# HySonLab/Protein_Redesign

Hardware: AMD Instinct MI355X
Metric: denoising-steps/sec (fwd+rev) per complex, N=256 res (higher is better)
Workload: dtype f32; 1 GPU; configs[1]: synthetic 256-residue + 64-atom ligand (N=320), single_dim=512 pair_dim=64 num_blocks=4 num_steps=1000, 1 complex/GPU, sharded by sample index (no data-path collective; one all_gather of the samples at the end of the timed region); samples_per_gpu=1, hip_graph=True, outputs_finite=True, backend=single process

## Files before the change

### protein_redesign_amd/csrc/prd_tri.hip

```cpp
#include "prd_common.h"
#include "../../include/prd_hip.h"
#include <atomic>
#include <cstdlib>
#include <cstring>
#include "prd_launch.h"

#ifdef PRD_TIMING
__device__ unsigned long long prd_dbg[256 * 16 * 8 * 4];
__device__ int prd_dbg_sel;
extern "C" int prd_debug_read(void* dst) { return (int)hipMemcpyFromSymbol(dst, HIP_SYMBOL(prd_dbg), sizeof(prd_dbg)); }
extern "C" int prd_debug_select(int id) { return (int)hipMemcpyToSymbol(HIP_SYMBOL(prd_dbg_sel), &id, sizeof(int)); }
#define PRD_STAMP(k) do { if (lane == 0 && it < 8) prd_dbg[((blockIdx.x * 12 + wave) * 8 + it) * 4 + (k)] = __builtin_readcyclecounter(); } while (0)
struct PhaseTimer {
    unsigned long long t, acc[8];
    __device__ PhaseTimer() { for (int k = 0; k < 8; ++k) acc[k] = 0; t = __builtin_readcyclecounter(); }
    __device__ void mark(int k) {
        __builtin_amdgcn_sched_barrier(0);
        const unsigned long long n = __builtin_readcyclecounter();
        __builtin_amdgcn_sched_barrier(0);
        acc[k] += n - t;
        t = n;
    }
    __device__ void flush(int id = 0) {
        if (prd_dbg_sel != 0 && prd_dbg_sel != id) return;
        if ((threadIdx.x & 63) == 0) for (int k = 0; k < 8; ++k) prd_dbg[(blockIdx.x * 16 + (threadIdx.x >> 6)) * 8 + k] = acc[k];
    }
};
#else
#define PRD_STAMP(k)
struct PhaseTimer {
    __device__ void mark(int) {}
    __device__ void flush(int = 0) {}
};
#endif

namespace {

struct ProjTask {
    int ob, vb, bb, u, bu;
    bool ok;
};
template <int OB>
PRD_DEV ProjTask proj_decode(long task, int nrb, int nvb, int N) {
    ProjTask t;
    const int ti = task < 0 ? 0 : (int)task;
    const int grp = ti / (8 * OB), within = ti % (8 * OB);
    t.ob = within >> 3;
    int rb = grp * 8 + (within & 7);
    t.ok = task >= 0 && rb < nrb;
    if (!t.ok) rb = 0;
    t.vb = rb % nvb;
    t.bu = rb / nvb;
    t.bb = t.bu / N;
    t.u = t.bu - t.bb * N;
    return t;
}
template <int P>
PRD_DEV void proj_fetch(const ProjTask& t, const float* __restrict__ pair, const float* __restrict__ mask, int N, int incoming,
                        int r, int hi, float (&x)[P / 2], float& mu, float& mv) {
    const int v = t.vb * 32 + r;
    const bool valid = v < N;
    const int vv = valid ? v : 0;
    mu = mask[t.bu];
    mv = mask[t.bb * N + vv];
    const prd_rsrc rs = make_rsrc(pair + (long)t.bb * N * N * P);
    const unsigned rowi = incoming ? (unsigned)vv * N + t.u : (unsigned)t.u * N + vv;
    load_row_cll_buf<P>(rs, valid ? (rowi * P + 4 * hi) * 4u : BUF_OOB, x);
}

template <int P, bool B3>
PRD_DEV void proj_compute(const ProjTask& t, float (&x)[P / 2], float mu, float mv, float* __restrict__ AB,
                          const float* Wpl, const float* Wgl, const float* bpl, const float* bgl,
                          int N, int ldn, long cstride, unsigned lane_off, int r, int hi, PhaseTimer& pt) {
    constexpr int KH = P / 2, OUT = 2 * P;
    const bool valid = t.vb * 32 + r < N;
    pt.mark(0);
    const float m2 = valid ? mu * mv : 0.f;
    const bool plain = __all(m2 == 1.0f);
    pt.mark(1);
    ln_cll<KH>(x);
    pt.mark(2);
    f32x16 ap[1], ag[1];
    bias_acc(ap, bpl + hi * P + 16 * t.ob);
    bias_acc(ag, bgl + hi * P + 16 * t.ob);
    if (B3) {
        u32x4 xs[2][P / 16];
        split2h_cll<KH>(x, xs);
        rowgemm_h2<P, 1>(reinterpret_cast<const u32x4*>(Wpl), OUT, t.ob * 32, xs, ap, r, hi);
        rowgemm_h2<P, 1>(reinterpret_cast<const u32x4*>(Wgl), OUT, t.ob * 32, xs, ag, r, hi);
#pragma unroll
        for (int q = 0; q < 16; ++q) { ap[0][q] *= H2_INV_WSCALE; ag[0][q] *= H2_INV_WSCALE; }
    } else {
        rowgemm<P, 1>(Wpl + t.ob * 32 * (P + 4), x, ap, r, hi);
        rowgemm<P, 1>(Wgl + t.ob * 32 * (P + 4), x, ag, r, hi);
    }
    pt.mark(3);
    const prd_rsrc cb = make_rsrc(AB + ((((long)t.bb * 2 * P) + 32 * t.ob) * N + t.u) * ldn + t.vb * 32);
    const unsigned cbytes = (unsigned)cstride * 4u;
    if (plain) {
#pragma unroll
        for (int q = 0; q < 16; q += 2) {
            const f32x2 den = f32x2{__builtin_amdgcn_exp2f(ag[0][q]), __builtin_amdgcn_exp2f(ag[0][q + 1])} + 1.0f;
            const f32x2 val = f32x2{ap[0][q], ap[0][q + 1]} * f32x2{__builtin_amdgcn_rcpf(den.x), __builtin_amdgcn_rcpf(den.y)};
            buf_store(val.x, cb, lane_off, ((q & 3) + 8 * (q >> 2)) * cbytes);
            buf_store(val.y, cb, lane_off, (((q + 1) & 3) + 8 * ((q + 1) >> 2)) * cbytes);
        }
    } else {
#pragma unroll
        for (int q = 0; q < 16; ++q)
            buf_store(m2 * (gate_from_scaled(ag[0][q]) * ap[0][q]), cb, lane_off, ((q & 3) + 8 * (q >> 2)) * cbytes);
    }
    pt.mark(4);
}

size_t tri_mul_proj_lds_bytes(int P, bool b3) { return (2 * (b3 ? (size_t)2 * P * P : (size_t)2 * P * (P + 4)) + 4 * P) * sizeof(float); }
template <int P, int NW, bool B3>
__global__ __launch_bounds__(NW * 64) void tri_mul_proj_kernel(int* queue, float* __restrict__ AB, const float* __restrict__ pair,
                                                          const float* __restrict__ mask,
                                                          const float* __restrict__ wp, const float* __restrict__ bp,
                                                          const float* __restrict__ wg, const float* __restrict__ bg,
                                                          int b, int N, int ldn, int incoming) {
    constexpr int KH = P / 2, OUT = 2 * P, OB = OUT / 32;
    extern __shared__ __attribute__((aligned(16))) float smem[];
    PhaseTimer pt;
    constexpr int WSZ = B3 ? OUT * P : OUT * (P + 4);
    float* Wpl = smem;
    float* Wgl = Wpl + WSZ;
    float* bpl = Wgl + WSZ;
    float* bgl = bpl + OUT;
    if (B3) {
        stage_weight_h2<P>(reinterpret_cast<u32x4*>(Wpl), wp, OUT, P, threadIdx.x, NW * 64, H2_WSCALE);
        stage_weight_h2<P>(reinterpret_cast<u32x4*>(Wgl), wg, OUT, P, threadIdx.x, NW * 64, NEG_LOG2E * H2_WSCALE);
    } else {
        stage_weight_cll<P>(Wpl, wp, OUT, P, threadIdx.x, NW * 64);
        stage_weight_cll<P>(Wgl, wg, OUT, P, threadIdx.x, NW * 64, NEG_LOG2E);
    }
    stage_vec_cll(bpl, bp, OUT, threadIdx.x, NW * 64, B3 ? H2_WSCALE : 1.0f);
    stage_vec_cll(bgl, bg, OUT, threadIdx.x, NW * 64, NEG_LOG2E * (B3 ? H2_WSCALE : 1.0f));
    const int lane = threadIdx.x & 63, r = lane & 31, hi = lane >> 5;
    const int nvb = ldn / 32;
    const int nrb = b * N * nvb;
    const long ntask = (long)((nrb + 7) / 8 * 8) * OB;
    const long cstride = (long)N * ldn;
    const unsigned lane_off = (hi * 4 * (unsigned)cstride + r) * 4u;
    WaveTasks tasks(queue, ntask, NW);
    float xa[KH], xb[KH], mua, mva, mub, mvb;
    long t = tasks.next();
    ProjTask ta = proj_decode<OB>(t, nrb, nvb, N), tb;
    proj_fetch<P>(ta, pair, mask, N, incoming, r, hi, xa, mua, mva);
    __syncthreads();
    pt.mark(6);
    while (t >= 0) {
        const long tn = tasks.next();
        tb = proj_decode<OB>(tn, nrb, nvb, N);
        proj_fetch<P>(tb, pair, mask, N, incoming, r, hi, xb, mub, mvb);
        if (ta.ok) proj_compute<P, B3>(ta, xa, mua, mva, AB, Wpl, Wgl, bpl, bgl, N, ldn, cstride, lane_off, r, hi, pt);
        if (tn < 0) break;
        t = tasks.next();
        ta = proj_decode<OB>(t, nrb, nvb, N);
        proj_fetch<P>(ta, pair, mask, N, incoming, r, hi, xa, mua, mva);
        if (tb.ok) proj_compute<P, B3>(tb, xb, mub, mvb, AB, Wpl, Wgl, bpl, bgl, N, ldn, cstride, lane_off, r, hi, pt);
    }
    pt.mark(5);
    pt.flush(1);
}

size_t tri_mul_out_proj_lds_bytes(int P) { return ((size_t)2 * P * P + (size_t)2 * 2 * P * P + 6 * P) * sizeof(float); }
template <int P, int NW>
__global__ __launch_bounds__(NW * 64) void tri_mul_out_proj_kernel(float* pair, const float* __restrict__ Ot, const float* __restrict__ mask,
                                                                   const float* __restrict__ wo, const float* __restrict__ bo,
                                                                   const float* __restrict__ wog, const float* __restrict__ bog,
                                                                   const float* __restrict__ wp, const float* __restrict__ bp,
                                                                   const float* __restrict__ wg, const float* __restrict__ bg,
                                                                   float* __restrict__ AB, int b, int N, int ldn) {
    constexpr int KH = P / 2, NB = P / 32, OUT = 2 * P, OB = OUT / 32;
    extern __shared__ __attribute__((aligned(16))) float smem_op[];
    float* Wol = smem_op;
    float* Wgol = Wol + P * P;
    float* Wpl = Wgol + P * P;
    float* Wgl = Wpl + OUT * P;
    float* bol = Wgl + OUT * P;
    float* bgol = bol + P;
    float* bpl = bgol + P;
    float* bgl = bpl + OUT;
    stage_weight_h2<P>(reinterpret_cast<u32x4*>(Wol), wo, P, P, threadIdx.x, NW * 64, H2_WSCALE);
    stage_weight_h2<P>(reinterpret_cast<u32x4*>(Wgol), wog, P, P, threadIdx.x, NW * 64, H2_WSCALE);
    stage_weight_h2<P>(reinterpret_cast<u32x4*>(Wpl), wp, OUT, P, threadIdx.x, NW * 64, H2_WSCALE);
    stage_weight_h2<P>(reinterpret_cast<u32x4*>(Wgl), wg, OUT, P, threadIdx.x, NW * 64, NEG_LOG2E * H2_WSCALE);
    stage_vec_cll(bol, bo, P, threadIdx.x, NW * 64);
    stage_vec_cll(bgol, bog, P, threadIdx.x, NW * 64);
    stage_vec_cll(bpl, bp, OUT, threadIdx.x, NW * 64, H2_WSCALE);
    stage_vec_cll(bgl, bg, OUT, threadIdx.x, NW * 64, NEG_LOG2E * H2_WSCALE);
    __syncthreads();
    const int lane = threadIdx.x & 63, r_w = lane & 31, hi_w = lane >> 5;
    const int nvb = ldn / 32;
    const long ntask = (long)b * N * nvb;
    const unsigned cbytes = (unsigned)N * (unsigned)ldn * 4u;
    WaveTasks tasks(nullptr, ntask, NW);
    for (long task = tasks.next(); task >= 0; task = tasks.next()) {
        int r = r_w, hi = hi_w;
        asm volatile("" : "+v"(r), "+v"(hi));
        const unsigned lane_off = (unsigned)(4 * hi) * cbytes + (unsigned)r * 4u;
        const int ti = (int)task;
        const int vb = ti % nvb, bu = ti / nvb;
        const int bb = bu / N, u = bu - bb * N;
        const int v = vb * 32 + r;
        const bool valid = v < N;
        const int vv = valid ? v : 0;
        float x[KH], xr[KH];
        {
            const prd_rsrc ro = make_rsrc(Ot + (((long)bb * P) * N + u) * ldn + vb * 32);
#pragma unroll
            for (int s = 0; s < KH; ++s) x[s] = buf_load(ro, valid ? lane_off : BUF_OOB, (unsigned)(8 * (s >> 2) + (s & 3)) * cbytes);
            const prd_rsrc rp = make_rsrc(pair + (long)bb * N * N * P);
            load_row_cll_buf<P>(rp, valid ? (((unsigned)vv * N + u) * P + 4 * hi) * 4u : BUF_OOB, xr);
        }
        const float mu = mask[bu], mv = mask[bb * N + vv];
        float gate[KH];
        {
            float xn[KH];
#pragma unroll
            for (int s = 0; s < KH; ++s) xn[s] = xr[s];
            ln_cll<KH>(xn);
            f32x16 ag[NB];
            zero_acc(ag);
            u32x4 xs[2][P / 16];
            split2h_cll<KH>(xn, xs);
            rowgemm_h2<P, NB>(reinterpret_cast<const u32x4*>(Wgol), P, 0, xs, ag, r, hi);
#pragma unroll
            for (int s = 0; s < KH; ++s) gate[s] = sigmoid_fast(ag[s >> 4][s & 15] * H2_INV_WSCALE + bgol[hi * KH + s]);
        }
        ln_cll<KH>(x);
        {
            f32x16 ao[NB];
            zero_acc(ao);
            u32x4 xs[2][P / 16];
            split2h_cll<KH>(x, xs);
            rowgemm_h2<P, NB>(reinterpret_cast<const u32x4*>(Wol), P, 0, xs, ao, r, hi);
#pragma unroll
            for (int s = 0; s < KH; ++s) x[s] = xr[s] + gate[s] * (ao[s >> 4][s & 15] * H2_INV_WSCALE + bol[hi * KH + s]);
        }
        store_row_cll<P>(pair + (((long)bb * N + vv) * N + u) * P, hi, valid, x);
        ln_cll<KH>(x);
        u32x4 xs[2][P / 16];
        split2h_cll<KH>(x, xs);
        const float m2 = valid ? mu * mv : 0.f;
        const bool plain = __all(m2 == 1.0f);
#pragma unroll
        for (int ob = 0; ob < OB; ++ob) {
            f32x16 ap[1], ag[1];
            bias_acc(ap, bpl + hi * P + 16 * ob);
            bias_acc(ag, bgl + hi * P + 16 * ob);
            rowgemm_h2<P, 1>(reinterpret_cast<const u32x4*>(Wpl), OUT, ob * 32, xs, ap, r, hi);
            rowgemm_h2<P, 1>(reinterpret_cast<const u32x4*>(Wgl), OUT, ob * 32, xs, ag, r, hi);
            const prd_rsrc cb = make_rsrc(AB + ((((long)bb * 2 * P) + 32 * ob) * N + u) * ldn + vb * 32);
            if (plain) {
#pragma unroll
                for (int q = 0; q < 16; ++q) {
                    const float val = (ap[0][q] * H2_INV_WSCALE) * gate_from_scaled(ag[0][q] * H2_INV_WSCALE);
                    buf_store(val, cb, lane_off, (unsigned)((q & 3) + 8 * (q >> 2)) * cbytes);
                }
            } else {
#pragma unroll
                for (int q = 0; q < 16; ++q)
                    buf_store(m2 * ((ap[0][q] * H2_INV_WSCALE) * gate_from_scaled(ag[0][q] * H2_INV_WSCALE)), cb, lane_off,
                              (unsigned)((q & 3) + 8 * (q >> 2)) * cbytes);
            }
        }
    }
}

__global__ __launch_bounds__(256) void tri_mul_contract_kernel(float* __restrict__ O, const float* __restrict__ AB,
                                                               int N, int ldn, int P, int nbatch, int tiles) {
    constexpr int KCH = 32, LDP = KCH + 4;
    __shared__ __attribute__((aligned(16))) float As[2][64 * LDP];
    __shared__ __attribute__((aligned(16))) float Bs[2][64 * LDP];
    const int tid = threadIdx.x, lane = tid & 63, wave = tid >> 6;
    const int r = lane & 31, hi = lane >> 5;
    const int wm0 = (wave >> 1) * 32, wn0 = (wave & 1) * 32;
    const int nch = nbatch * P;
    const int t2 = tiles * tiles;
    for (int vblk = blockIdx.x; vblk < nch * t2; vblk += gridDim.x) {
    int ch, tile;
    if ((nch & 7) == 0 && (gridDim.x & 7) == 0) {
        const int xcd = vblk & 7, k = vblk >> 3;
        ch = xcd + 8 * (k / t2);
        tile = k % t2;
    } else {
        ch = vblk / t2;
        tile = vblk % t2;
    }
    const int bb = ch / P, d = ch - bb * P;
    const int m0 = (tile / tiles) * 64, n0 = (tile % tiles) * 64;
    const float* __restrict__ A = AB + ((size_t)bb * 2 * P + d) * N * ldn;
    const float* __restrict__ B = AB + ((size_t)bb * 2 * P + P + d) * N * ldn;
    const int srow = tid >> 3, sf = tid & 7;
    const bool a0 = (m0 + srow) < N, a1 = (m0 + srow + 32) < N, b0 = (n0 + srow) < N, b1 = (n0 + srow + 32) < N;
    const prd_rsrc ra = make_rsrc(A + (size_t)m0 * ldn), rb = make_rsrc(B + (size_t)n0 * ldn);
    const unsigned oa0 = a0 ? ((unsigned)srow * ldn + 4 * sf) * 4u : BUF_OOB, oa1 = a1 ? ((unsigned)(srow + 32) * ldn + 4 * sf) * 4u : BUF_OOB;
    const unsigned ob0 = b0 ? ((unsigned)srow * ldn + 4 * sf) * 4u : BUF_OOB, ob1 = b1 ? ((unsigned)(srow + 32) * ldn + 4 * sf) * 4u : BUF_OOB;
    f32x16 acc;
#pragma unroll
    for (int q = 0; q < 16; ++q) acc[q] = 0.f;
    const int nchunk = ldn / KCH;
#define PRD_TMC_LD1(RS, OFF, KO) [&] { const auto v_ = __builtin_amdgcn_raw_buffer_load_b128(RS, OFF, (KO) * 4, 0);      \
        return make_float4(__uint_as_float(v_[0]), __uint_as_float(v_[1]), __uint_as_float(v_[2]), __uint_as_float(v_[3])); }()
#define PRD_TMC_LOAD(R, KO)                                                       \
    R##a0 = PRD_TMC_LD1(ra, oa0, KO);                                             \
    R##a1 = PRD_TMC_LD1(ra, oa1, KO);                                             \
    R##b0 = PRD_TMC_LD1(rb, ob0, KO);                                             \
    R##b1 = PRD_TMC_LD1(rb, ob1, KO);
#define PRD_TMC_STAGE(R, BUF)                                                     \
    *reinterpret_cast<float4*>(&As[BUF][srow * LDP + 4 * sf]) = R##a0;            \
    *reinterpret_cast<float4*>(&As[BUF][(srow + 32) * LDP + 4 * sf]) = R##a1;     \
    *reinterpret_cast<float4*>(&Bs[BUF][srow * LDP + 4 * sf]) = R##b0;            \
    *reinterpret_cast<float4*>(&Bs[BUF][(srow + 32) * LDP + 4 * sf]) = R##b1;
#define PRD_TMC_CHUNK(C, CUR, R, N)                                               \
    {                                                                             \
        const int c2 = (C) + 2 < nchunk ? (C) + 2 : nchunk - 1;                   \
        PRD_TMC_LOAD(N, c2 * KCH)                                                 \
        const float* as = &As[CUR][(wm0 + r) * LDP + hi * 16];                    \
        const float* bs = &Bs[CUR][(wn0 + r) * LDP + hi * 16];                    \
        _Pragma("unroll") for (int t = 0; t < 4; ++t) {                           \
            const float4 a = *reinterpret_cast<const float4*>(as + 4 * t);        \
            const float4 bq = *reinterpret_cast<const float4*>(bs + 4 * t);       \
            acc = mfma32(a.x, bq.x, acc);                                         \
            acc = mfma32(a.y, bq.y, acc);                                         \
            acc = mfma32(a.z, bq.z, acc);                                         \
            acc = mfma32(a.w, bq.w, acc);                                         \
        }                                                                         \
        if ((C) + 1 < nchunk) { PRD_TMC_STAGE(R, (CUR) ^ 1) }                     \
        __syncthreads();                                                          \
    }
    float4 ua0, ua1, ub0, ub1, va0, va1, vb0, vb1;
    PRD_TMC_LOAD(u, 0)
    PRD_TMC_STAGE(u, 0)
    {
        const int c1 = 1 < nchunk ? 1 : 0;
        PRD_TMC_LOAD(u, c1 * KCH)
    }
    __syncthreads();
    for (int c = 0; c < nchunk; c += 2) {
        PRD_TMC_CHUNK(c, 0, u, v)
        if (c + 1 < nchunk) PRD_TMC_CHUNK(c + 1, 1, v, u)
    }
#undef PRD_TMC_LOAD
#undef PRD_TMC_LD1
#undef PRD_TMC_STAGE
#undef PRD_TMC_CHUNK
    float* __restrict__ Oc = O + (size_t)ch * N * ldn;
    const int n = n0 + wn0 + r;
    if (n < N) {
#pragma unroll
        for (int q = 0; q < 16; ++q) {
            const int m = m0 + wm0 + drow32(q, hi);
            if (m < N) Oc[(size_t)m * ldn + n] = acc[q];
        }
    }
    }
}

constexpr int TMS_T = 160, TMS_PLANE = TMS_T * 64, TMS_OPER = 2 * TMS_PLANE;
size_t tri_mul_contract_split_lds_bytes() { return (size_t)4 * TMS_OPER; }
template <int NWV, int DEPTH = 2, bool ASC = false>
__global__ __launch_bounds__(NWV * 64) void tri_mul_contract_split_kernel(float* __restrict__ O, const float* __restrict__ AB,
                                                                          int N, int ldn, int P, int nbatch, int tiles, int swap,
                                                                          const unsigned* __restrict__ a_amax) {
    constexpr int NT = NWV * 64, NPT = (2560 + NT - 1) / NT, NSUB = (25 + NWV - 1) / NWV;
    extern __shared__ __attribute__((aligned(16))) unsigned char tms[];
    PhaseTimer pt;
    const int tid = threadIdx.x, lane = tid & 63, wave = tid >> 6;
    const int r = lane & 31, hi = lane >> 5;
    const int nch = nbatch * P;
    const int t2 = tiles * tiles;
    unsigned srow[NPT], sdst[NPT], ssrc[NPT];
    bool sisb[NPT], sok[NPT];
    const int wbase = __builtin_amdgcn_readfirstlane(tid & ~63);
#pragma unroll
    for (int i = 0; i < NPT; ++i) {
        const int pw = wbase + NT * i;
        sok[i] = pw < 2560;
        const int oper = (sok[i] && pw >= 1280) ? 1 : 0;
        const int pc = sok[i] ? tid + NT * i : 0;
        const int q = pc - 1280 * oper;
        const int row = q >> 3, f = q & 7;
        sisb[i] = oper == 1;
        srow[i] = row;
        sdst[i] = oper * TMS_OPER + row * 64 + (((f >> 1) ^ ((row >> 2) & 3)) << 4) + (f & 1) * 8;
        ssrc[i] = ((unsigned)row * ldn + 4 * f) * 4u;
    }
    const unsigned swz = (unsigned)((r >> 2) & 3);
    for (int vblk = blockIdx.x; vblk < nch * t2; vblk += gridDim.x) {
        int ch, tile;
        if ((nch & 7) == 0 && (gridDim.x & 7) == 0) {
            const int xcd = vblk & 7, k = vblk >> 3;
            ch = xcd + 8 * (k / t2);
            tile = k % t2;
        } else {
            ch = vblk / t2;
            tile = vblk % t2;
        }
        const int bb = ch / P, d = ch - bb * P;
        const int m0 = (tile / tiles) * TMS_T, n0 = (tile % tiles) * TMS_T;
        float asc = 1.0f, iasc = 1.0f;
        if constexpr (ASC) {
            asc = split_scale(a_amax[bb]);
            iasc = __uint_as_float((254u << 23) - __float_as_uint(asc));
        }
        const float* __restrict__ A = AB + ((size_t)bb * 2 * P + (swap ? P : 0) + d) * N * ldn;
        const float* __restrict__ B = AB + ((size_t)bb * 2 * P + (swap ? 0 : P) + d) * N * ldn;
        const prd_rsrc ra = make_rsrc(A + (size_t)m0 * ldn), rb = make_rsrc(B + (size_t)n0 * ldn);
        unsigned off[NPT];
#pragma unroll
        for (int i = 0; i < NPT; ++i)
            off[i] = (sok[i] && (sisb[i] ? n0 : m0) + (int)srow[i] < N) ? ssrc[i] : BUF_OOB;
        int si[NSUB], sj[NSUB];
        bool sv[NSUB];
#pragma unroll
        for (int k = 0; k < NSUB; ++k) {
            const int s_ = wave + NWV * k;
            si[k] = s_ / 5;
            sj[k] = s_ - 5 * si[k];
            sv[k] = s_ < 25 && m0 + 32 * si[k] < N && n0 + 32 * sj[k] < N;
        }
        f32x16 acc[NSUB];
        zero_acc(acc);
        const int nchunk = ldn / 32;
        u32x4 u[NPT], v[NPT];
#define PRD_TMS_LOAD(R, C)                                                                                          \
    _Pragma("unroll") for (int i = 0; i < NPT; ++i)                                                                 \
        R[i] = __builtin_bit_cast(u32x4, __builtin_amdgcn_raw_buffer_load_b128(sisb[i] ? rb : ra, off[i], (C) * 128, 0));
#define PRD_TMS_STAGE(R, BUF)                                                                                       \
    _Pragma("unroll") for (int i = 0; i < NPT; ++i) {                                                               \
        if (!sok[i]) continue;                                                                                      \
        float x0 = __uint_as_float(R[i][0]), x1 = __uint_as_float(R[i][1]), x2 = __uint_as_float(R[i][2]), x3 = __uint_as_float(R[i][3]); \
        if (ASC && !sisb[i]) { x0 *= asc; x1 *= asc; x2 *= asc; x3 *= asc; }                                       \
        unsigned h0, l0, h1, l1;                                                                                    \
        split2h(x0, x1, h0, l0);                                                                                    \
        split2h(x2, x3, h1, l1);                                                                                    \
        unsigned char* dst = tms + (BUF) * 2 * TMS_OPER + sdst[i];                                                  \
        *reinterpret_cast<u32x2*>(dst) = u32x2{h0, h1};                                                             \
        *reinterpret_cast<u32x2*>(dst + TMS_PLANE) = u32x2{l0, l1};                                                 \
    }
#define PRD_TMS_CHUNK(C, CUR, R, NX)                                                                                \
    {                                                                                                               \
        const int c2 = (C) + 2 < nchunk ? (C) + 2 : nchunk - 1;                                                     \
        PRD_TMS_LOAD(NX, c2)                                                                                        \
        const unsigned char* base = tms + (CUR) * 2 * TMS_OPER;                                                     \
        _Pragma("unroll") for (int st = 0; st < 2; ++st) {                                                          \
            const unsigned col = (((unsigned)(2 * st + hi)) ^ swz) << 4;                                            \
            _Pragma("unroll") for (int k = 0; k < NSUB; ++k) {                                                      \
                if (sv[k]) {                                                                                        \
                    const unsigned char* ap = base + (32 * si[k] + r) * 64 + col;                                   \
                    const unsigned char* bp = base + TMS_OPER + (32 * sj[k] + r) * 64 + col;                        \
                    u32x4 a[2], bq[2];                                                                              \
                    _Pragma("unroll") for (int pl = 0; pl < 2; ++pl) {                                              \
                        a[pl] = *reinterpret_cast<const u32x4*>(ap + pl * TMS_PLANE);                               \
                        bq[pl] = *reinterpret_cast<const u32x4*>(bp + pl * TMS_PLANE);                              \
                    }                                                                                               \
                    const int pa[3] = {0, 0, 1}, pb[3] = {0, 1, 0};                                                 \
                    _Pragma("unroll") for (int t = 0; t < 3; ++t)                                                   \
                        acc[k] = __builtin_amdgcn_mfma_f32_32x32x16_f16(__builtin_bit_cast(f16x8_t, a[pa[t]]),      \
                                                                        __builtin_bit_cast(f16x8_t, bq[pb[t]]), acc[k], 0, 0, 0); \
                }                                                                                                   \
// ... 1693 lines not shown
```

Baseline: 597.4 denoising-steps/s.

## Process whole row-blocks across all output blocks in triangle projection, split only the tail

The triangle-multiplication projection previously split every row block into OB separate tasks, one per 32-wide output block. Each task re-fetched the pair row, redid the LayerNorm and the fp16 split. Now most tasks cover all output blocks for a row, reusing the normalized input, and only the leftover rows that do not fill a full round of wave slots are split per output block to balance the tail. This cuts redundant global loads and LayerNorm work, at the cost of longer tasks and the lane index being recomputed from mbcnt inline asm.

```diff
diff --git a/protein_redesign_amd/csrc/prd_tri.hip b/protein_redesign_amd/csrc/prd_tri.hip
--- a/protein_redesign_amd/csrc/prd_tri.hip
+++ b/protein_redesign_amd/csrc/prd_tri.hip
@@ -37,16 +37,23 @@
 namespace {
 
 struct ProjTask {
-    int ob, vb, bb, u, bu;
+    int ob0, ob1, vb, bb, u, bu;
     bool ok;
 };
+constexpr int PROJ_PIECE_ROUNDS = 1;
 template <int OB>
-PRD_DEV ProjTask proj_decode(long task, int nrb, int nvb, int N) {
+PRD_DEV ProjTask proj_decode(long task, int nwhole, int nrb, int nvb, int N) {
     ProjTask t;
     const int ti = task < 0 ? 0 : (int)task;
-    const int grp = ti / (8 * OB), within = ti % (8 * OB);
-    t.ob = within >> 3;
-    int rb = grp * 8 + (within & 7);
+    int rb = ti;
+    t.ob0 = 0;
+    t.ob1 = OB;
+    if (ti >= nwhole) {
+        const int q = ti - nwhole, grp = q / (8 * OB), within = q % (8 * OB);
+        t.ob0 = within >> 3;
+        t.ob1 = t.ob0 + 1;
+        rb = nwhole + grp * 8 + (within & 7);
+    }
     t.ok = task >= 0 && rb < nrb;
     if (!t.ok) rb = 0;
     t.vb = rb % nvb;
@@ -55,9 +62,15 @@
     t.u = t.bu - t.bb * N;
     return t;
 }
+PRD_DEV int proj_lane() {
+    int lane;
+    asm volatile("v_mbcnt_lo_u32_b32 %0, -1, 0\n\tv_mbcnt_hi_u32_b32 %0, -1, %0" : "=v"(lane));
+    return lane;
+}
 template <int P>
 PRD_DEV void proj_fetch(const ProjTask& t, const float* __restrict__ pair, const float* __restrict__ mask, int N, int incoming,
-                        int r, int hi, float (&x)[P / 2], float& mu, float& mv) {
+                        float (&x)[P / 2], float& mu, float& mv) {
+    const int lane = proj_lane(), r = lane & 31, hi = lane >> 5;
     const int v = t.vb * 32 + r;
     const bool valid = v < N;
     const int vv = valid ? v : 0;
@@ -69,48 +82,60 @@
 }
 
 template <int P, bool B3>
+PRD_DEV void proj_block(const ProjTask& t, int ob, const float (&x)[P / 2], const u32x4 (&xs)[2][P / 16], float m2, bool plain,
+                        float* __restrict__ AB, const float* Wpl, const float* Wgl, const float* bpl, const float* bgl,
+                        int N, int ldn, long cstride, unsigned lane_off, int r, int hi, PhaseTimer& pt) {
+    constexpr int OUT = 2 * P;
+    f32x16 ap[1], ag[1];
+    bias_acc(ap, bpl + hi * P + 16 * ob);
+    bias_acc(ag, bgl + hi * P + 16 * ob);
+    if (B3) {
+        rowgemm_h2<P, 1>(reinterpret_cast<const u32x4*>(Wpl), OUT, ob * 32, xs, ap, r, hi);
+        rowgemm_h2<P, 1>(reinterpret_cast<const u32x4*>(Wgl), OUT, ob * 32, xs, ag, r, hi);
+#pragma unroll
+        for (int q = 0; q < 16; ++q) { ap[0][q] *= H2_INV_WSCALE; ag[0][q] *= H2_INV_WSCALE; }
+    } else {
+        rowgemm<P, 1>(Wpl + ob * 32 * (P + 4), x, ap, r, hi);
+        rowgemm<P, 1>(Wgl + ob * 32 * (P + 4), x, ag, r, hi);
+    }
+    pt.mark(3);
+    const prd_rsrc cb = make_rsrc(AB + ((((long)t.bb * 2 * P) + 32 * ob) * N + t.u) * ldn + t.vb * 32);
+    const unsigned cbytes = (unsigned)cstride * 4u;
+    if (plain) {
+#pragma unroll
+        for (int q = 0; q < 16; q += 2) {
+            const f32x2 den = f32x2{__builtin_amdgcn_exp2f(ag[0][q]), __builtin_amdgcn_exp2f(ag[0][q + 1])} + 1.0f;
+            const f32x2 val = f32x2{ap[0][q], ap[0][q + 1]} * f32x2{__builtin_amdgcn_rcpf(den.x), __builtin_amdgcn_rcpf(den.y)};
+            buf_store(val.x, cb, lane_off, ((q & 3) + 8 * (q >> 2)) * cbytes);
+            buf_store(val.y, cb, lane_off, (((q + 1) & 3) + 8 * ((q + 1) >> 2)) * cbytes);
+        }
+    } else {
+#pragma unroll
+        for (int q = 0; q < 16; ++q)
+            buf_store(m2 * (gate_from_scaled(ag[0][q]) * ap[0][q]), cb, lane_off, ((q & 3) + 8 * (q >> 2)) * cbytes);
+    }
+    pt.mark(4);
+}
+
+template <int P, bool B3>
 PRD_DEV void proj_compute(const ProjTask& t, float (&x)[P / 2], float mu, float mv, float* __restrict__ AB,
                           const float* Wpl, const float* Wgl, const float* bpl, const float* bgl,
-                          int N, int ldn, long cstride, unsigned lane_off, int r, int hi, PhaseTimer& pt) {
-    constexpr int KH = P / 2, OUT = 2 * P;
+                          int N, int ldn, long cstride, PhaseTimer& pt) {
+    constexpr int KH = P / 2;
+    const int lane = proj_lane(), r = lane & 31, hi = lane >> 5;
+    const unsigned lane_off = (hi * 4 * (unsigned)cstride + r) * 4u;
     const bool valid = t.vb * 32 + r < N;
     pt.mark(0);
     const float m2 = valid ? mu * mv : 0.f;
     const bool plain = __all(m2 == 1.0f);
     pt.mark(1);
     ln_cll<KH>(x);
+    u32x4 xs[2][P / 16];
+    if (B3) split2h_cll<KH>(x, xs);
     pt.mark(2);
-    f32x16 ap[1], ag[1];
-    bias_acc(ap, bpl + hi * P + 16 * t.ob);
-    bias_acc(ag, bgl + hi * P + 16 * t.ob);
-    if (B3) {
-        u32x4 xs[2][P / 16];
-        split2h_cll<KH>(x, xs);
-        rowgemm_h2<P, 1>(reinterpret_cast<const u32x4*>(Wpl), OUT, t.ob * 32, xs, ap, r, hi);
-        rowgemm_h2<P, 1>(reinterpret_cast<const u32x4*>(Wgl), OUT, t.ob * 32, xs, ag, r, hi);
-#pragma unroll
-        for (int q = 0; q < 16; ++q) { ap[0][q] *= H2_INV_WSCALE; ag[0][q] *= H2_INV_WSCALE; }
-    } else {
-        rowgemm<P, 1>(Wpl + t.ob * 32 * (P + 4), x, ap, r, hi);
-        rowgemm<P, 1>(Wgl + t.ob * 32 * (P + 4), x, ag, r, hi);
-    }
-    pt.mark(3);
-    const prd_rsrc cb = make_rsrc(AB + ((((long)t.bb * 2 * P) + 32 * t.ob) * N + t.u) * ldn + t.vb * 32);
-    const unsigned cbytes = (unsigned)cstride * 4u;
-    if (plain) {
-#pragma unroll
-        for (int q = 0; q < 16; q += 2) {
-            const f32x2 den = f32x2{__builtin_amdgcn_exp2f(ag[0][q]), __builtin_amdgcn_exp2f(ag[0][q + 1])} + 1.0f;
-            const f32x2 val = f32x2{ap[0][q], ap[0][q + 1]} * f32x2{__builtin_amdgcn_rcpf(den.x), __builtin_amdgcn_rcpf(den.y)};
-            buf_store(val.x, cb, lane_off, ((q & 3) + 8 * (q >> 2)) * cbytes);
-            buf_store(val.y, cb, lane_off, (((q + 1) & 3) + 8 * ((q + 1) >> 2)) * cbytes);
-        }
-    } else {
-#pragma unroll
-        for (int q = 0; q < 16; ++q)
-            buf_store(m2 * (gate_from_scaled(ag[0][q]) * ap[0][q]), cb, lane_off, ((q & 3) + 8 * (q >> 2)) * cbytes);
-    }
-    pt.mark(4);
+#pragma unroll 1
+    for (int ob = t.ob0; ob < t.ob1; ++ob)
+        proj_block<P, B3>(t, ob, x, xs, m2, plain, AB, Wpl, Wgl, bpl, bgl, N, ldn, cstride, lane_off, r, hi, pt);
 }
 
 size_t tri_mul_proj_lds_bytes(int P, bool b3) { return (2 * (b3 ? (size_t)2 * P * P : (size_t)2 * P * (P + 4)) + 4 * P) * sizeof(float); }
@@ -137,29 +162,33 @@
     }
     stage_vec_cll(bpl, bp, OUT, threadIdx.x, NW * 64, B3 ? H2_WSCALE : 1.0f);
     stage_vec_cll(bgl, bg, OUT, threadIdx.x, NW * 64, NEG_LOG2E * (B3 ? H2_WSCALE : 1.0f));
-    const int lane = threadIdx.x & 63, r = lane & 31, hi = lane >> 5;
     const int nvb = ldn / 32;
     const int nrb = b * N * nvb;
-    const long ntask = (long)((nrb + 7) / 8 * 8) * OB;
+    int nwhole = nrb;
+    if (!queue) {
+        const int slots = (int)gridDim.x * NW, left = nrb % slots;
+        const int npiece = (left + 7) / 8 * 8 * OB;
+        if (npiece <= PROJ_PIECE_ROUNDS * slots) nwhole = nrb - left;
+    }
+    const long ntask = (long)nwhole + (long)((nrb - nwhole + 7) / 8 * 8) * OB;
     const long cstride = (long)N * ldn;
-    const unsigned lane_off = (hi * 4 * (unsigned)cstride + r) * 4u;
     WaveTasks tasks(queue, ntask, NW);
     float xa[KH], xb[KH], mua, mva, mub, mvb;
     long t = tasks.next();
-    ProjTask ta = proj_decode<OB>(t, nrb, nvb, N), tb;
-    proj_fetch<P>(ta, pair, mask, N, incoming, r, hi, xa, mua, mva);
+    ProjTask ta = proj_decode<OB>(t, nwhole, nrb, nvb, N), tb;
+    proj_fetch<P>(ta, pair, mask, N, incoming, xa, mua, mva);
     __syncthreads();
     pt.mark(6);
     while (t >= 0) {
         const long tn = tasks.next();
-        tb = proj_decode<OB>(tn, nrb, nvb, N);
-        proj_fetch<P>(tb, pair, mask, N, incoming, r, hi, xb, mub, mvb);
-        if (ta.ok) proj_compute<P, B3>(ta, xa, mua, mva, AB, Wpl, Wgl, bpl, bgl, N, ldn, cstride, lane_off, r, hi, pt);
+        tb = proj_decode<OB>(tn, nwhole, nrb, nvb, N);
+        proj_fetch<P>(tb, pair, mask, N, incoming, xb, mub, mvb);
+        if (ta.ok) proj_compute<P, B3>(ta, xa, mua, mva, AB, Wpl, Wgl, bpl, bgl, N, ldn, cstride, pt);
         if (tn < 0) break;
         t = tasks.next();
-        ta = proj_decode<OB>(t, nrb, nvb, N);
-        proj_fetch<P>(ta, pair, mask, N, incoming, r, hi, xa, mua, mva);
-        if (tb.ok) proj_compute<P, B3>(tb, xb, mub, mvb, AB, Wpl, Wgl, bpl, bgl, N, ldn, cstride, lane_off, r, hi, pt);
+        ta = proj_decode<OB>(t, nwhole, nrb, nvb, N);
+        proj_fetch<P>(ta, pair, mask, N, incoming, xa, mua, mva);
+        if (tb.ok) proj_compute<P, B3>(tb, xb, mub, mvb, AB, Wpl, Wgl, bpl, bgl, N, ldn, cstride, pt);
     }
     pt.mark(5);
     pt.flush(1);
```

After: 604.2 denoising-steps/s (median of 6 runs). +1.2%, better.
